# OpenMatchmaking/microservice-matchmaking

Measured on AMD Instinct MI355X. Metric: matched players/sec over 1M-player pool, higher is better.
Workload: dtype int32

## Files before the change

### microservice_matchmaking_amd/csrc/mm_engine.hip

```cpp
#include <hip/hip_runtime.h>

#include <stdint.h>
#include <stdio.h>
#include <stdlib.h>
#include <string.h>
#include <time.h>

#include <dlfcn.h>

#include <algorithm>
#include <mutex>
#include <cmath>
#include <new>
#include <vector>

#include "../../include/mm_engine.h"
#include "../../include/mm_wait.h"
#include <mm_gfx950.h>


#define MM_NO_SLOT 0xFFFFFFFFu
#define MM_ST_FREE 0
#define MM_ST_LIVE 1
#define MM_ST_CANCELLED 2
// ... 2103 lines not shown
            last_tp = tp;
            for (uint32_t g = 0; g < G; ++g) P.pyq[g] = 0;
            P.pyq[yield_g] = yield_q;
            {
                P.grp = (e->tn.pair_group_min && tiles >= e->tn.pair_group_min && tp == PK_TMAX) ? PK_GS : 0u;
                const uint32_t ngr = P.grp ? (tiles + P.grp - 1u) / P.grp : 0u;
                dim3 rgrid(tiles, G);
                P.xslots = 0;
                uint32_t tof[MM_MAX_GROUPS];
                for (uint32_t g = 0; g < G; ++g) tof[g] = P.bm[g] ? (P.bm[g] + tp - 1u) / tp : 0u;
                if (persist) {
                    const uint32_t slots = pair_xcd_map(P, tof, G, true);
                    if (slots) {
                        P.grp = 0;
                        const uint32_t K = e->tn.pair_pbatch, slice = MM_PERSIST_SLICE ? MM_PERSIST_SLICE : K + 1u;
                        for (uint32_t it = 0; it <= K; it += slice)
                            TILE_LAUNCH(kp_rounds, dim3(8u * slots), dim3(PT_THREADS), P, it, it + slice < K + 1u ? it + slice : K + 1u, K);
                        ++e->ps.pair_rounds_launches;
                        after_persist = true;
                        COMPACT_LAUNCH();
                        HIPCHK(e, hipGetLastError());
                        MMTRY(results_absorb(e, M.L));
                        MMTRY(results_send(e, sent_no, M.L, e->tn.results_early ? MM_RESULTS_MIN_PAIR : 0xFFFFFFFFu));
                        continue;
                    }
                    P.xslots = 0;
                }
                if (e->tn.pair_xcd) {
                    const uint32_t slots = pair_xcd_map(P, tof, G);
                    if (slots) rgrid = dim3(8u * slots);
                }
                uint32_t r = e->round_ctr;
                TILE_LAUNCH(kp_round, rgrid, dim3(PT_THREADS), P, r, 1u);
                ++r;
                if (P.grp) TILE_LAUNCH(kp_group, dim3(ngr, G), dim3(1024), P, r);
                for (uint32_t b = 0; b < (want_fit && e->tn.pair_batch > 12u ? 12u : e->tn.pair_batch); ++b) {
                    TILE_LAUNCH(kp_round, rgrid, dim3(PT_THREADS), P, r, 0u);
                    ++e->ps.pair_round_launches;
                    ++r;
                    if (P.grp) TILE_LAUNCH(kp_group, dim3(ngr, G), dim3(1024), P, r);
                }
                TILE_LAUNCH(kp_round_commit, dim3(tiles, G), dim3(256), P, r);
                hipLaunchKernelGGL(kp_round_stage, dim3(G), dim3(64), 0, e->stream, P, r);
                COMPACT_LAUNCH();
                e->round_ctr = r;
            }
#undef COMPACT_LAUNCH
#undef TILE_LAUNCH
            HIPCHK(e, hipGetLastError());
            MMTRY(results_absorb(e, M.L));
            MMTRY(results_send(e, sent_no, M.L, e->tn.results_early ? MM_RESULTS_MIN_PAIR : 0xFFFFFFFFu));
        }
    }
    hipLaunchKernelGGL(kp_late, dim3(G), dim3(PL_THREADS), 0, e->stream, P);
    hipLaunchKernelGGL(kp_finish, dim3(G), dim3(1024), 0, e->stream, P);
    HIPCHK(e, hipGetLastError());
    if (tail_send) {
        MMTRY(results_absorb(e, M.L));
        MMTRY(results_send(e, tail_no, M.L, e->tn.results_early ? MM_RESULTS_MIN_PAIR : 0xFFFFFFFFu));
    }
    return MM_OK;
}

static void report_team(const mm_engine* e)
{
    const uint32_t G = e->cfg.n_groups;
    for (uint32_t g = 0; g < G; ++g) {
        const TeamChain& t = e->h_tchains[g];
        const uint32_t np = t.passes + 1u;
        fprintf(stderr, "[mm-team] g%u fast %u m %u passes %u out %u left %u | cancel tick: head sat out %u, seated %u, lobby filtered %u, anchor moved %u x | "
                "kt_f, the middle chunk, cycles per pass: first loads %u, probes + lists %u, replacements %u, look-ups from scratch %u, barrier %u, step C %u; anchors at work per pass %u | "
                "F values written %u, changed after the first pass %u | kt_chase: sub-queue entries looked at by the stored lobby's fills %u, by %u look-ups %u\n",
                g, t.fast, t.m, t.passes, t.n_out, t.qlen,
                t.dbg[6] & 1u, (t.dbg[6] >> 1) & 1u, (t.dbg[6] >> 2) & 1u, t.dbg[7],
                t.tmk[0] / np, t.tmk[1] / np, t.tmk[2] / np, t.tmk[3] / np, t.tmk[4] / np, t.tmk[5] / np, t.dbg[2] / np, t.dbg[5], t.dbg[4],
                t.dbg[0], t.dbg[3], t.dbg[1]);
        if (t.lt[11])
            fprintf(stderr, "[mm-team] g%u kt_fc's chaser: %u passes, %u lobbies by F; cycles per pass: all %u, the chase loop %u, its hops by F %u, of them on kt_f's flags %u; "
                    "cycles per hop without the flags %u; %u look-ups, cycles each: starts %u, the roles' stretches %u, the members' records %u, seats + kills (the one a pass ends on) %u "
                    "(with MM_TEAM_LATE=0: kt_late keeps its own timers in the same words)\n",
                    g, t.lt[11], t.lt[12], 16u * (t.lt[9] / t.lt[11]), 16u * (t.lt[10] / t.lt[11]), 16u * (t.lt[13] / t.lt[11]), 16u * (t.lt[8] / t.lt[11]),
                    t.lt[12] ? (uint32_t)(16ull * (t.lt[13] - t.lt[8]) / t.lt[12]) : 0u,
                    t.lt[3], t.lt[3] ? 16u * (t.lt[4] / t.lt[3]) : 0u, t.lt[3] ? 16u * (t.lt[5] / t.lt[3]) : 0u, t.lt[3] ? 16u * (t.lt[6] / t.lt[3]) : 0u,
                    16u * (t.lt[7] / t.lt[11]));
    }
}

static void report_team_late(const mm_engine* e, const uint32_t* p0)
{
    const uint32_t G = e->cfg.n_groups;
    for (uint32_t g = 0; g < G; ++g) {
        const TeamChain& t = e->h_tchains[g];
        if (t.fast && t.passes != p0[g])
            fprintf(stderr, "[mm-team-late] g%u: kt_late walked passes %u..%u%s (m %u, sub-queues %u %u %u %u %u): "
                    "%u lobbies by record, %u looked up, %u left open, %u stored fills; entries scanned per role %u %u %u %u %u; "
                    "cycles/16: records %u look-ups %u fills %u ring waits %u all %u\n", g, p0[g], t.passes,
                    t.done ? "" : " and handed the chain back", t.m, t.len[0], t.len[1], t.len[2], t.len[3], t.len[4],
                    t.lt[1], t.lt[2], t.lt[3], t.lt[4], t.lt[5], t.lt[6], t.lt[7], t.lt[8], t.lt[9], t.lt[10], t.lt[11],
                    t.lt[12], t.lt[14], t.lt[13]);
    }
}

static void report_team_pass(mm_engine* e, uint32_t guard)
{
    const uint32_t G = e->cfg.n_groups;
    uint32_t gl = 0;
    for (uint32_t g = 1; g < G; ++g)
// ... 142 lines not shown
        ++e->ps.host_looks;
        {
            uint32_t fl = 0;
            for (uint32_t g = 0; g < G; ++g) if (e->h_tchains[g].fast) fl += e->h_tchains[g].flags_late;
            e->ps.team_flags_late = fl;
        }
        bool busy = false, late = late_ok;
        uint32_t most = 0;
        for (uint32_t g = 0; g < G; ++g) {
            const TeamChain& t = e->h_tchains[g];
            if (!t.fast || t.done) continue;
            busy = true;
            most = t.n_vis > most ? t.n_vis : most;
            if (t.n_vis > e->tn.team_late) late = false;
        }
        if (e->tn.debug && late_now) report_team_late(e, p0);
        if (e->tn.debug && e->tn.team_batch == 1u && !late_now) report_team_pass(e, guard);
        {
            uint32_t bf[MM_MAX_GROUPS];
            for (uint32_t g = 0; g < G; ++g) { bf[g] = e->h_tchains[g].before; team_no[g] = e->h_tchains[g].fast ? e->h_tchains[g].n_out : 0u; }
            if (!e->r_based) results_set_bases(e, bf, M.L);
            team_have = true;
        }
        if (!busy) break;
        team_order();
        if (late_now) {
            late_now = false;
            if (pass < 2u) pass = 2u;
            batch = e->tn.team_batch;
            continue;
        }
        late_now = late;
        n_emit = most / (TT_WAVES - 1u) + 1u;
        if (n_emit > e->tn.team_emit_max) n_emit = e->tn.team_emit_max;
        batch = (e->tn.team_late && most <= 3u * e->tn.team_late) ? (e->tn.team_batch < 4u ? e->tn.team_batch : 4u) : e->tn.team_batch;
    }
    if (e->ps.team_flags_late) { e->ps.team_flags_late_total += e->ps.team_flags_late; e->ps.degraded = 1; }
    hipLaunchKernelGGL(kt_fin_scatter, dim3(nch, G), dim3(TT_CH), 0, e->stream, P);
    hipLaunchKernelGGL(kt_fin_copy, dim3(nch, G), dim3(TT_CH), 0, e->stream, P);
    HIPCHK(e, hipGetLastError());
    if (e->tn.debug) report_team(e);
    return MM_OK;
}

static int report_pair(mm_engine* e)
{
    const uint32_t G = e->cfg.n_groups;
    std::vector<PairChain> hp(G);
    HIPCHK(e, hipMemcpy(hp.data(), e->d_pchains, G * sizeof(PairChain), hipMemcpyDeviceToHost));
    for (uint32_t g = 0; g < G; ++g)
        fprintf(stderr, "[mm-pair] g%u fast %u m %u qlen %u passes %u out %u rounds %u (group hops of tile 0: %u of %u entries looked at, %u not of the round) | stale %u inv %u slowsucc %u compact %u fixed(w1) %u | chase clk %u wall(100MHz) %u wrapscan clk %u\n",
                g, hp[g].fast, hp[g].m, hp[g].qlen, hp[g].passes, hp[g].n_out, hp[g].rounds, hp[g].ghops, hp[g].gtry, hp[g].gstale, hp[g].dbg[0], hp[g].dbg[1],
                hp[g].dbg[2], hp[g].dbg[3], hp[g].dbg[4], hp[g].dbg[5], hp[g].dbg[6], hp[g].dbg[7]);
    for (uint32_t g = 0; g < G; ++g)
        if (hp[g].rounds) {
            const uint32_t nr = hp[g].tm[5] ? hp[g].tm[5] : 1u;
            fprintf(stderr, "[mm-pair] g%u tile1 cycles/round over %u rounds (load %u walk+stage+sweepA %u apply %u | detect %u items %u long %u (%.1f long items) | graph %u resolve %u publish %u | cand+head %u)\n",
                    g, nr, hp[g].tm[0] / nr, hp[g].tm[6] / nr, hp[g].tm[9] / nr, hp[g].tm[1] / nr, hp[g].tm[12] / nr, hp[g].tm[2] / nr,
                    (double)hp[g].tm[11] / nr, hp[g].tm[7] / nr, hp[g].tm[8] / nr, hp[g].tm[10] / nr, hp[g].tm[4] / nr);
        }
    for (uint32_t g = 0; g < G; ++g)
        if (hp[g].ppass) {
            const uint32_t nr = hp[g].ptm[5] ? hp[g].ptm[5] : 1u;
            fprintf(stderr, "[mm-pair] g%u kp_rounds: %u passes inside persistent launches (%u launches gave up so far); tile1 cycles/pass over %u passes (barrier %u fast hops %u walk+sweepA %u apply %u | detect %u items %u long %u | graph %u resolve %u publish %u | head+arrive %u) walk loop %.0f cycles, %.1f hops\n",
                    g, hp[g].ppass, e->pair_pstops, nr, hp[g].ptm[0] / nr, hp[g].ptm[3] / nr, hp[g].ptm[6] / nr, hp[g].ptm[9] / nr, hp[g].ptm[1] / nr,
                    hp[g].ptm[12] / nr, hp[g].ptm[2] / nr, hp[g].ptm[7] / nr, hp[g].ptm[8] / nr, hp[g].ptm[10] / nr, hp[g].ptm[4] / nr,
                    16.0 * hp[g].ptm[13] / nr, (double)hp[g].ptm[15] / nr);
            fprintf(stderr, "[mm-pair] g%u kp_rounds, tile 1's walker off the fast path: %u hops whose partner had left, %.0f cycles each; %u hops without a partner inside the horizon, %.0f cycles each\n",
                    g, hp[g].pslow[0], hp[g].pslow[0] ? 16.0 * hp[g].pslow[1] / hp[g].pslow[0] : 0.0, hp[g].pslow[2],
                    hp[g].pslow[2] ? 16.0 * hp[g].pslow[3] / hp[g].pslow[2] : 0.0);
        }
    {
        fprintf(stderr, "[mm-pair] physical XCD mask of each chain's workgroups in its last kp_rounds launch:");
        for (uint32_t g = 0; g < G; ++g) fprintf(stderr, " g%u=0x%x", g, hp[g].pxm);
        fprintf(stderr, " | key %p rec %p %p bitsp %p %p pbar %p stream %p\n", (void*)e->d_pk_key[0], (void*)e->d_pk_scratch, (void*)e->d_pk_rec1,
                (void*)e->d_pk_bitsp[0], (void*)e->d_pk_bitsp[1], (void*)e->d_pk_pbar, (void*)e->stream);
    }
    if (e->tn.pair_tune & 0x10000u) {
        const uint32_t nt = 40u;
        std::vector<uint4> dg(nt);
        for (uint32_t g = 0; g < G; ++g) {
            if (!hp[g].ppass) continue;
            HIPCHK(e, hipMemcpy(dg.data(), e->d_pk_grec + (size_t)g * e->pk_gstride, nt * sizeof(uint4), hipMemcpyDeviceToHost));
            fprintf(stderr, "[mm-pair] g%u kp_rounds, cycles from barrier to arrival per tile (passes):", g);
            for (uint32_t t = 0; t < nt; ++t) if (dg[t].y && dg[t].y != 0xFFFFFFFFu) fprintf(stderr, " t%u=%u(%u)", t, dg[t].x / dg[t].y, dg[t].y);
            fprintf(stderr, "\n");
        }
    }
    if (e->tn.pair_tune & 0x2000u) {
        unsigned long long tested = 0, algo = 0;
        for (uint32_t g = 0; g < G; ++g) { tested += hp[g].tested; algo += hp[g].pairs; }
        fprintf(stderr, "[mm-pair] predicate tests the kernels physically performed (next[] build, repairs, head scans, LDS-resident walk): %llu = %.2f x the %llu pair evaluations of the reference algorithm\n",
                tested, algo ? (double)tested / (double)algo : 0.0, algo);
        std::vector<uint32_t> xc(e->pk_max_tiles);
        HIPCHK(e, hipMemcpy(xc.data(), e->d_pk_tilectl + ((size_t)TC_DISP * G + 0) * e->pk_max_tiles,
                            e->pk_max_tiles * sizeof(uint32_t), hipMemcpyDeviceToHost));
        fprintf(stderr, "[mm-pair] g0 XCD of tile 0..47's workgroup at its last round:");
        for (uint32_t t = 0; t < 48 && t < e->pk_max_tiles; ++t) fprintf(stderr, " %u", xc[t] & 0xFu);
        fprintf(stderr, "\n");
    }
    if (e->tn.pair_tune & 0x2000u)
        for (uint32_t g = 0; g < G; ++g)
            if (hp[g].rounds)
                fprintf(stderr, "[mm-pair] g%u walk loop of tile 1's workgroup: %u iterations, %.0f cycles each (%.0f cycles per timed round)\n",
                        g, hp[g].tm[15], hp[g].tm[15] ? 16.0 * hp[g].tm[13] / hp[g].tm[15] : 0.0,
                        16.0 * hp[g].tm[13] / (hp[g].tm[5] ? hp[g].tm[5] : 1u));
// ... 1078 lines not shown
```

### microservice_matchmaking_amd/csrc/mm_pair.inc

```

#define PK_NO 0xFFFFFFFFu
#define PK_ABORT 0xFFFFFFFEu

#define NX_INV 0u
#define NX_NONE 0xFFFFu
#define NX_FAR 0xFFFEu

#ifndef PK_T
#define PK_T 8192u
#endif
enum : uint32_t { PK_TMAX = PK_T };
#undef PK_T
static constexpr uint32_t PK_T = PK_TMAX;
#ifndef PK_TILES_MAX
#define PK_TILES_MAX 40u
#endif
#define PK_XSEG 4u
#ifndef PK_GS
#define PK_GS 8u
#endif
#ifndef PK_GROUP_MIN
#define PK_GROUP_MIN 64u
#endif
#ifndef PL_MAX
// ... 19 lines not shown
#define DISP_SEATED 0xFFFFFFFEu
#define REC_CLEAN 0u
#define REC_PARTNER 1u
#define REC_FAR 2u
#define REC_NONE 3u
#define EV_NONE 0u
#define EV_DONE 1u
#define EV_COMPACT 2u

struct RoundState {
    uint32_t live;
    uint32_t done;
    uint32_t want_compact, rounds;
    uint32_t qlen, passes, n_out, has_anchor;
    uint32_t a_key, a_slot, a_cons, a_team;
    int32_t  a_rating;
    uint32_t pos0;
    uint32_t changed0, extra0;
    uint32_t a_oi;
    unsigned long long pairs, scanned;
};

struct PairChain {
    uint32_t fast;
    uint32_t m;
    uint32_t qlen;
    uint32_t buf;
    int32_t  rmin;
    uint32_t has_anchor;
    uint32_t a_key, a_slot, a_cons, a_team;
    int32_t  a_rating;
    uint32_t passes, n_out, before, err;
    uint32_t pos0;
    uint32_t changed0;
    uint32_t extra0;
    unsigned long long pairs, scanned;
    unsigned long long tested;
    unsigned long long tested_nx;
    uint32_t dbg[8];
    uint32_t stage;
    uint32_t ntiles;
    uint32_t want_compact;
    uint32_t cur_pass;
    uint32_t new_m;
    uint32_t rounds;
    uint32_t ghops;
    uint32_t gtry, gstale;
    uint32_t tm[16];
    uint32_t pfail;
    uint32_t ppass;
    uint32_t pxm;
    uint32_t pslow[4];
    uint32_t ptm[16];
    RoundState rs[2];
};

struct PairParams {
    uint32_t mode, n_groups, capacity, window, eqmask;
    uint32_t out_slot_stride, out_rec_stride, bits_stride;
    uint32_t pstride;
    uint32_t tune;
    uint32_t purge;
    uint8_t* state;
    uint32_t* released;
    uint32_t* n_released;
    ChainDev* chains;
    PairChain* pchains;
    int32_t* q_rating;
    uint32_t* q_cons;
    uint32_t* q_slot;
    uint32_t* key[2];
    uint32_t* oidx[2];
    uint16_t* nx16[2];
    uint32_t* bits[2];
    uint32_t* scratch;
    uint16_t* g16;
    uint32_t* rec2[2];
    uint16_t* exa[2];
    uint32_t* bitsp[2];
    uint32_t* headp[2];
    uint4* grec;
    uint32_t grp;
    uint32_t xslots;
    uint32_t xseg[8][PK_XSEG];
    uint16_t xcnt[8][PK_XSEG];
    uint32_t gstride;
    unsigned long long* pbar;
    uint32_t* pxmask;
    uint32_t ptimeout0, ptimeout1;
    uint32_t pinject;
    uint32_t* pyield;
    uint32_t pyq[MM_MAX_GROUPS];
    uint16_t* wpre;
    uint32_t* tilectl;
    uint32_t max_tiles;
    uint32_t* out_slots;
    float* out_score;
    uint32_t* out_pass;
    uint32_t bm[MM_MAX_GROUPS];
    uint8_t bbuf[MM_MAX_GROUPS];
};

#define PK_DEAD 0x80000000u
#define PK_SPAN_BITS 19
#define PK_RMASK 0x7FFFFu
static __device__ __forceinline__ uint32_t pk_pack(int32_t r, uint32_t cons, int32_t rmin, uint32_t eqmask)
// ... 71 lines not shown
        bool fast = lb.n <= 1u && m <= max_len;
        if (m + has > 0 && ((long long)hi - (long long)lo) >= (1ll << PK_SPAN_BITS)) fast = false;
        if (m + has == 0) lo = 0;
        uint32_t pos0 = 0, changed0 = 0, extra0 = 0;
        if (fast && P.purge && has) {
            const uint32_t hs = ch->head_state;
            const uint32_t stale_slot = a_slot;
            if (hs != 0u && P.state[stale_slot] != MM_ST_LIVE) {
                if (hs == 1u) {
                    const size_t qo = (size_t)c * P.capacity;
                    const int32_t hr = qr[0];
                    const uint32_t hc = P.q_cons[qo];
                    const uint32_t d = hr >= a_rating ? (uint32_t)hr - (uint32_t)a_rating : (uint32_t)a_rating - (uint32_t)hr;
                    pos0 = 1;
                    if (d <= P.window && (((hc ^ a_cons) & P.eqmask) == 0u)) {
                        extra0 = 1; changed0 = 1;
                        a_slot = P.q_slot[qo]; a_rating = hr; a_cons = hc; team = 1u - team;
                    } else has = 0;
                } else has = 0;
                P.state[stale_slot] = MM_ST_FREE;
                P.released[atomicAdd(P.n_released, 1u)] = stale_slot;
            }
        }
        pc->fast = fast ? 1u : 0u;
        pc->m = m;
        pc->qlen = m - extra0;
        pc->pos0 = pos0;
        pc->changed0 = changed0;
        pc->extra0 = extra0;
        pc->buf = 0;
        pc->rmin = lo;
        pc->has_anchor = has;
        pc->a_key = has ? pk_pack(a_rating, a_cons, lo, P.eqmask) : 0u;
        pc->a_slot = a_slot;
        pc->a_cons = a_cons;
        pc->a_team = team;
        pc->a_rating = a_rating;
        pc->passes = 0;
        pc->n_out = 0;
        pc->before = m + lb.n + (P.purge ? ch->purged : 0u);
        pc->err = 0;
        pc->pairs = 0;
        pc->scanned = 0;
        pc->tested = 0;
        pc->tested_nx = 0;
        for (int k = 0; k < 8; ++k) pc->dbg[k] = 0;
        pc->stage = m < PL_MAX ? PS_LATE : PS_TILED;
        pc->ntiles = (m + PK_T - 1u) / PK_T;
        pc->want_compact = 0;
        pc->cur_pass = 0;
        pc->new_m = m;
        pc->rounds = 0;
        pc->ghops = 0; pc->gtry = 0; pc->gstale = 0;
        for (int k = 0; k < 16; ++k) { pc->tm[k] = 0; pc->ptm[k] = 0; }
        pc->pfail = 0; pc->ppass = 0;
        for (int k = 0; k < 4; ++k) pc->pslow[k] = 0;
        pc->pxm = 0;
        P.pbar[g] = 0ull; P.pxmask[g] = 0u;
        if (g == 0u) *P.pyield = 0u;
    }
    if (m <= max_len) {
        const uint32_t nt = (m + PK_T - 1u) / PK_T;
        for (uint32_t t = tid; t < P.max_tiles; t += 1024) {
            P.tilectl[((size_t)TC_ENT * P.n_groups + g) * P.max_tiles + t] = PK_NO;
            P.tilectl[((size_t)TC_ALIVE * P.n_groups + g) * P.max_tiles + t] =
                t < nt ? dev_min_u32(PK_T, m - t * PK_T) : 0u;
        }
    }
}

__global__ __launch_bounds__(1024) void kp_pack(PairParams P)
{
    const uint32_t g = blockIdx.y;
    const PairChain* const pc = P.pchains + g;
    if (!pc->fast) return;
    const uint32_t m = pc->m;
    const uint32_t i = blockIdx.x * 1024u + threadIdx.x;
    const uint32_t c = P.mode * P.n_groups + g;
    const size_t qo = (size_t)c * P.capacity, po = (size_t)g * P.pstride;
    if (i < m) {
        P.key[0][po + i] = pk_pack(P.q_rating[qo + i], P.q_cons[qo + i], pc->rmin, P.eqmask);
        P.oidx[0][po + i] = i;
        P.nx16[0][po + i] = (uint16_t)NX_INV;
    }
    if ((i & 31u) == 0u && i < m + 32u) {
        const uint32_t left = i < m ? m - i : 0u;
        uint32_t wbits = left >= 32u ? 0xFFFFFFFFu : ((1u << left) - 1u);
        if (i == 0u && pc->extra0) wbits &= ~1u;
        P.bits[0][(size_t)g * P.bits_stride + (i >> 5)] = wbits;
    }
}

#define NXI_THREADS 512
#define NXI_SEG 2048u
#define NXI_STAGE 8192u
__global__ __launch_bounds__(NXI_THREADS) void kp_nx_init(PairParams P, uint32_t seg, uint32_t stage)
{
    __shared__ uint32_t s_k[NXI_STAGE];
    const uint32_t g = blockIdx.y;
    const PairChain* const pc = P.pchains + g;
    if (!pc->fast) return;
    const uint32_t m = pc->m;
    const uint32_t s0 = blockIdx.x * seg;
    if (s0 >= m) return;
    const int tid = threadIdx.x, lane = tid & 63, wave = tid >> 6;
    const size_t po = (size_t)g * P.pstride;
    const uint32_t* const key = P.key[0] + po;
// ... 90 lines not shown
        for (; p + 256u <= end; p += 256u) {
            uint32_t kv[4];
#pragma unroll
            for (uint32_t u = 0; u < 4u; ++u) kv[u] = lds_ld(key + p + 64u * u + (uint32_t)lane);
#pragma unroll
            for (uint32_t u = 0; u < 4u; ++u) {
                const unsigned long long b = __ballot(pk_in(kv[u], klo, krng));
                if (b) return p + 64u * u + (uint32_t)__ffsll(b) - 1u;
            }
        }
    }
    if (ev) {
        for (; p + 256u <= end; p += 256u) {
            uint32_t kv[4];
#pragma unroll
            for (uint32_t u = 0; u < 4u; ++u) kv[u] = lds_ld(key + p + 64u * u + (uint32_t)lane);
            const uint32_t e = lds_ld(ev);
#pragma unroll
            for (uint32_t u = 0; u < 4u; ++u) {
                const unsigned long long b = __ballot(pk_in(kv[u], klo, krng));
                if (b) return p + 64u * u + (uint32_t)__ffsll(b) - 1u;
            }
            if (uni(e) != EV_NONE) return PK_ABORT;
        }
    }
    for (; p < end; p += 64u) {
        const uint32_t c = p + (uint32_t)lane;
        const bool ok = c < end && pk_in(lds_ld(key + c), klo, krng);
        const unsigned long long b = __ballot(ok);
        if (b) return p + (uint32_t)__ffsll(b) - 1u;
        if (ev && lds_ld(ev) != EV_NONE) return PK_ABORT;
    }
    return PK_NO;
}

static __device__ __forceinline__ uint32_t l_succ(const uint32_t* bits, uint32_t pos, uint32_t m, int lane)
{
    if (pos >= m) return PK_NO;
    const uint32_t nwords = (m + 31u) >> 5, w0 = pos >> 5;
    for (uint32_t wb = w0; wb < nwords; wb += 64u) {
        const uint32_t wi = wb + (uint32_t)lane;
        uint32_t v = wi < nwords ? lds_ld(bits + wi) : 0u;
        if (wi == w0) v &= 0xFFFFFFFFu << (pos & 31u);
        const unsigned long long b = __ballot(v != 0u);
        if (b) {
            const int l = __ffsll(b) - 1;
            const uint32_t vv = lane_get(v, l);
            return ((wb + (uint32_t)l) << 5) + (uint32_t)__ffs((int)vv) - 1u;
        }
    }
    return PK_NO;
}

#define PL_RING 512u
#define PL_EXT 0xFFFEu
#define PL_NOPART 0xFFFFu
#define PL_S (PL_MAX - 1u)
#define PL_SPEC 64u

static __device__ __forceinline__ uint32_t nxg_make(uint32_t t, uint32_t gi) { return t | ((gi << 2) << 16); }

static __device__ __forceinline__ uint32_t lane_succ(const uint32_t* bits, uint32_t from, uint32_t nwords)
{
    uint32_t wi = from >> 5;
    if (wi >= nwords) return PL_S;
    uint32_t v = lds_ld(bits + wi) & (0xFFFFFFFFu << (from & 31u));
    while (v == 0u) {
        if (++wi >= nwords) return PL_S;
        v = lds_ld(bits + wi);
    }
    return (wi << 5) + (uint32_t)__ffs((int)v) - 1u;
}

__global__ __launch_bounds__(PL_THREADS) void kp_late(PairParams P)
{
    __shared__ uint32_t s_path[PL_SPEC];
    __shared__ uint32_t s_nxg[PL_MAX];
    __shared__ uint32_t s_key[PL_MAX];
    __shared__ uint32_t s_bits[PL_WORDS + 64];
    __shared__ uint16_t s_wpre[PL_WORDS];
    __shared__ uint32_t s_ring[PL_RING];
    __shared__ uint16_t s_ringp[PL_RING];
    __shared__ uint32_t s_wtot[16];
    __shared__ uint32_t s_event, s_m, s_head, s_tail, s_killed, s_aidx, s_buf, s_nout;
    __shared__ uint32_t s_ext[5];

    const int tid = threadIdx.x, lane = tid & 63, wave = tid >> 6;
    const uint32_t g = blockIdx.x;
    PairChain* const pc = P.pchains + g;
    if (!pc->fast || pc->stage != PS_LATE) return;
    const uint32_t c = P.mode * P.n_groups + g;
    const size_t qo = (size_t)c * P.capacity, po = (size_t)g * P.pstride;
    const uint32_t w = P.window;
    uint32_t* const os = P.out_slots + (size_t)g * P.out_slot_stride;
    float* const osc = P.out_score + (size_t)g * P.out_rec_stride;
    uint32_t* const opass = P.out_pass + (size_t)g * P.out_rec_stride;
    uint32_t* const vbits = s_bits;
    uint32_t* const vev = &s_event;

    uint32_t m = pc->m;
    const uint32_t pass0 = pc->passes;
    {
        const uint32_t nwords = (m + 31u) >> 5;
        for (uint32_t i = tid; i < PL_WORDS + 64u; i += PL_THREADS)
            s_bits[i] = i < nwords ? P.bits[pc->buf][(size_t)g * P.bits_stride + i] : 0u;
        const uint32_t* const key = P.key[pc->buf] + po;
        __syncthreads();
        for (uint32_t i = tid; i < m; i += PL_THREADS) s_key[i] = key[i] | (l_alive(s_bits, i) ? 0u : PK_DEAD);
        if (tid == 0) {
            s_event = EV_NONE; s_m = m; s_head = 0; s_tail = 0; s_killed = 0; s_aidx = PK_NO; s_buf = pc->buf;
            s_ext[0] = pc->a_slot; s_ext[1] = (uint32_t)pc->a_rating; s_ext[2] = pc->a_cons;
            s_ext[3] = pc->a_key; s_ext[4] = pc->a_team;
        }
        __syncthreads();
        for (uint32_t i = tid; i < PL_MAX; i += PL_THREADS) {
            uint32_t t = LNX_NONE, gi = PL_S;
            if (i < m) {
                const uint32_t o = P.nx16[pc->buf][po + i];
                t = o == NX_NONE ? LNX_NONE : (o == NX_INV || o == NX_FAR) ? LNX_INV : i + o;
                if (t < LNX_INV) gi = lane_succ(s_bits, t + 1u, nwords);
            }
            s_nxg[i] = nxg_make(t, gi);
        }
    }
    __syncthreads();

    uint32_t has_anchor = pc->has_anchor, a_idx = PL_EXT, a_pushed = 1;
    uint32_t qlen = pc->qlen, pos = pc->pos0, passes = pc->passes, in_pass = pc->pos0 ? 1u : 0u, changed = pc->changed0;
    uint32_t n_out = pc->n_out;
    unsigned long long pairs = pc->pairs, scanned = pc->scanned;
    if (pc->pos0) { scanned += qlen + pc->extra0; pairs += qlen + pc->extra0; }
    uint32_t rk = 0, rtail = 0;
    uint32_t emit_idx = pc->n_out;
    uint32_t d_stale = 0, d_inv = 0, d_slowsucc = 0, d_compact = 0, d_fixed = 0, d_clk = 0, d_wall = 0, d_wrapc = 0;
    unsigned long long d_tst = 0;
    const uint32_t fix_waves = 13u - dev_min_u32(P.tune & 15u, 13u);
    const uint32_t fix_sleep = (P.tune >> 4) & 0xFFu;

#define RING_ROOM(N)                                                                        \
    do {                                                                                    \
        if (rk - rtail + (N) > PL_RING) {                                                   \
            rtail = uni(lds_ld(&s_tail));                                                   \
            while (rk - rtail + (N) > PL_RING) { __builtin_amdgcn_s_sleep(2); rtail = uni(lds_ld(&s_tail)); } \
        }                                                                                   \
    } while (0)
#define RING_PUSH(A, T)                                                                     \
    do {                                                                                    \
        RING_ROOM(1u);                                                                      \
        if (lane == 0) {                                                                    \
            s_ring[rk % PL_RING] = (A) | ((T) << 16);                                       \
            s_ringp[rk % PL_RING] = (uint16_t)(passes - pass0);                             \
        }                                                                                   \
        ++rk;                                                                               \
        if (lane == 0) lds_st(&s_head, rk);                                                 \
    } while (0)
#define RING_DRAIN()    \
    do {                                                                                    \
        uint32_t kd = uni(lds_ld(&s_killed));                                               \
        while (kd != rk) { __builtin_amdgcn_s_sleep(1); kd = uni(lds_ld(&s_killed)); }      \
    } while (0)

    for (;;) {
        if (wave == 0) {
            __builtin_amdgcn_s_setprio(3);
            uint32_t ev = EV_NONE;
            const long long tc0 = clock64(), tw0 = wall_clock64();
            for (;;) {
                if (!in_pass) {
                    RING_DRAIN();
                    if (qlen == 0u) { ev = EV_DONE; break; }
                    if (m > PL_COMPACT_MIN && qlen * 2u < m) { ev = EV_COMPACT; break; }
                    in_pass = 1; pos = 0; changed = 0;
                    scanned += qlen;
                    pairs += qlen;
                }
                uint32_t t = PK_NO;
                if (!has_anchor) {
                    const uint32_t a = uni(l_succ(vbits, pos, m, lane));
                    if (a == PK_NO) {
                        ++passes; in_pass = 0;
                        if (!changed) { ev = EV_DONE; break; }
                        continue;
                    }
                    --qlen; --pairs; changed = 1; has_anchor = 1; a_idx = a; a_pushed = 0;
                    pos = a + 1u;
                } else {
                    const long long ts = clock64();
                    const uint32_t a_key = a_idx == PL_EXT ? s_ext[3] : (s_key[a_idx] & ~PK_DEAD);
                    t = uni(l_scan_fit(s_key, a_key, pos, m, w, lane, nullptr));
                    d_tst += (t == PK_NO ? m : t) - pos;
                    d_wrapc += (uint32_t)(clock64() - ts);
                    if (t == PK_NO) {
                        ++passes; in_pass = 0;
                        if (!changed) { ev = EV_DONE; break; }
                        continue;
                    }
                }
                for (;;) {
                    bool blind = t == PK_NO && a_idx != PL_EXT;
                    if (blind) {
                        const uint32_t r0 = uni(lds_ld(s_nxg + a_idx));
                        blind = (r0 & 0xFFFFu) < LNX_INV && (r0 >> 18) != PL_S;
                    }
                    if (blind) {
                        uint32_t x4 = a_idx << 2;
                        for (uint32_t k0 = 0; k0 < PL_SPEC; k0 += 8u) {
#pragma unroll
                            for (uint32_t k = 0; k < 8u; ++k) {
                                const uint32_t r = lds_ld((const uint32_t*)((const char*)s_nxg + x4));
                                s_path[k0 + k] = r;
                                x4 = r >> 16;
                            }
                            if (uni(x4) == (PL_S << 2)) {
                                for (uint32_t k = k0 + 8u + (uint32_t)lane; k < PL_SPEC; k += 64u) s_path[k] = nxg_make(LNX_NONE, PL_S);
                                break;
                            }
                        }
                        const uint32_t r = s_path[lane];
                        const uint32_t rp = lane ? s_path[lane - 1] : 0u;
                        const uint32_t ia = lane ? (rp >> 18) : a_idx;
                        const uint32_t it = r & 0xFFFFu, ig = r >> 18;
                        bool ok = ia != PL_S && it < LNX_INV && ig != PL_S;
                        if (ok) ok = l_alive(vbits, it) && l_alive(vbits, ig);
                        const unsigned long long good = __ballot(ok);
                        const uint32_t ns = good == ~0ull ? 64u : (uint32_t)__ffsll(~good) - 1u;
                        if (ns) {
                            RING_ROOM(ns);
                            if ((uint32_t)lane < ns) {
                                s_ring[(rk + (uint32_t)lane) % PL_RING] = ia | (it << 16);
                                s_ringp[(rk + (uint32_t)lane) % PL_RING] = (uint16_t)(passes - pass0);
                            }
                            rk += ns;
                            if (lane == 0) lds_st(&s_head, rk);
                            qlen -= 2u * ns; pairs -= ns; n_out += ns; changed = 1;
                            a_idx = lane_get(ig, (int)ns - 1);
                            a_pushed = 0;
                        }
                        if (ns == PL_SPEC) continue;
                    }
                    const uint32_t a_key = a_idx == PL_EXT ? s_ext[3] : (s_key[a_idx] & ~PK_DEAD);
                    if (t == PK_NO) {
                        const uint32_t cnx = uni(lds_ld(s_nxg + a_idx)) & 0xFFFFu;
                        if (cnx == LNX_NONE) break;
                        if (cnx < LNX_INV && l_alive(vbits, cnx)) t = cnx;
                        else {
                            if (cnx == LNX_INV) ++d_inv; else ++d_stale;
                            t = uni(l_scan_fit(s_key, a_key, cnx == LNX_INV ? a_idx + 1u : cnx + 1u, m, w, lane, nullptr));
                            d_tst += (t == PK_NO ? m : t) - (cnx == LNX_INV ? a_idx + 1u : cnx + 1u);
                            if (t == PK_NO) break;
                        }
                    }
                    RING_PUSH(a_idx, t);
                    --qlen; changed = 1; has_anchor = 0; pos = t + 1u; ++n_out;
                    ++d_slowsucc;
                    const uint32_t a2 = uni(l_succ(vbits, t + 1u, m, lane));
                    if (a2 == PK_NO) break;
                    --qlen; --pairs; has_anchor = 1; a_idx = a2; a_pushed = 0;
                    pos = a2 + 1u;
                    t = PK_NO;
                }
                if (has_anchor && !a_pushed) { RING_PUSH(a_idx, PL_NOPART); a_pushed = 1; }
                ++passes; in_pass = 0;
                if (!changed) { ev = EV_DONE; break; }
            }
            d_clk += (uint32_t)(clock64() - tc0);
            d_wall += (uint32_t)(wall_clock64() - tw0);
            if (lane == 0) { s_aidx = has_anchor ? a_idx : PK_NO; s_nout = n_out; lds_st(vev, ev); }
            __builtin_amdgcn_s_setprio(0);
        } else if (wave == 1) {
            uint32_t ktail = uni(lds_ld(&s_killed));
            for (;;) {
                uint32_t head = uni(lds_ld(&s_head));
                if (head == ktail) {
                    if (lds_ld(vev) != EV_NONE) {
                        head = uni(lds_ld(&s_head));
                        if (head == ktail) break;
                    } else { __builtin_amdgcn_s_sleep(1); continue; }
                }
                const uint32_t nb = dev_min_u32(64u, head - ktail);
                if ((uint32_t)lane < nb) {
                    const uint32_t e = s_ring[(ktail + (uint32_t)lane) % PL_RING];
                    const uint32_t a = e & 0xFFFFu, t = e >> 16;
                    if (a != PL_EXT) { atomicAnd(&s_bits[a >> 5], ~(1u << (a & 31u))); atomicOr(&s_key[a], PK_DEAD); }
                    if (t != PL_NOPART) { atomicAnd(&s_bits[t >> 5], ~(1u << (t & 31u))); atomicOr(&s_key[t], PK_DEAD); }
                }
                wave_lockstep();
                ktail += nb;
                if (lane == 0) lds_st(&s_killed, ktail);
            }
        } else if (wave == 2) {
            uint32_t tail = uni(lds_ld(&s_tail));
            const uint32_t* const oidx = P.oidx[uni(lds_ld(&s_buf))] + po;
            for (;;) {
                const uint32_t killed = uni(lds_ld(&s_killed));
                if (killed == tail) {
                    if (lds_ld(vev) != EV_NONE && uni(lds_ld(&s_head)) == tail && uni(lds_ld(&s_killed)) == tail) break;
                    __builtin_amdgcn_s_sleep(2);
                    continue;
                }
                const uint32_t nb = dev_min_u32(64u, killed - tail);
                const bool mine = (uint32_t)lane < nb;
                const uint32_t slotr = (tail + (uint32_t)lane) % PL_RING;
                const uint32_t e = mine ? s_ring[slotr] : 0xFFFFFFFFu;
                const uint32_t a = e & 0xFFFFu, t = e >> 16;
                const bool is_match = mine && t != PL_NOPART;
                const unsigned long long mm = __ballot(is_match);
                if (is_match) {
                    const uint32_t k = emit_idx + (uint32_t)__popcll(mm & ((1ull << lane) - 1ull));
                    const uint32_t ka = a == PL_EXT ? s_ext[3] : s_key[a];
                    const uint32_t kt = s_key[t];
                    const uint32_t ra = pk_rating(ka), rt = pk_rating(kt);
                    const uint32_t team = a == PL_EXT ? s_ext[4] : 0u;
                    os[2u * k + team] = a == PL_EXT ? s_ext[0] : P.q_slot[qo + oidx[a]];
                    os[2u * k + (1u - team)] = P.q_slot[qo + oidx[t]];
                    osc[k] = (float)(int32_t)(ra > rt ? ra - rt : rt - ra);
// ... 75 lines not shown
        {
            const uint32_t nwords = (m + 31u) >> 5;
            const uint32_t pcw = (uint32_t)tid < nwords ? (uint32_t)__popc(s_bits[tid]) : 0u;
            const uint32_t incl = wave_incl_scan(pcw, lane);
            if (lane == 63) s_wtot[wave] = incl;
            __syncthreads();
            if ((uint32_t)tid < PL_WORDS) {
                uint32_t off = 0;
                for (int x = 0; x < wave; ++x) off += s_wtot[x];
                s_wpre[tid] = (uint16_t)(off + incl - pcw);
            }
            __syncthreads();
            uint32_t* const oidx_new = P.oidx[cur ^ 1u] + po;
            for (uint32_t base = 0; base < m; base += PL_THREADS) {
                const uint32_t i = base + (uint32_t)tid;
                uint32_t r = PK_NO, nk = 0, nv = 0, no = 0;
                if (i < m && l_alive(s_bits, i)) {
                    const uint32_t bw = s_bits[i >> 5];
                    r = s_wpre[i >> 5] + (uint32_t)__popc(bw & ((1u << (i & 31u)) - 1u));
                    nk = s_key[i];
                    const uint32_t v = s_nxg[i];
                    uint32_t t = v & 0xFFFFu, gi = v >> 18;
                    if (t < LNX_INV) {
                        if (l_alive(s_bits, t)) {
                            t = s_wpre[t >> 5] + (uint32_t)__popc(s_bits[t >> 5] & ((1u << (t & 31u)) - 1u));
                            if (gi != PL_S && l_alive(s_bits, gi))
                                gi = s_wpre[gi >> 5] + (uint32_t)__popc(s_bits[gi >> 5] & ((1u << (gi & 31u)) - 1u));
                            else gi = PL_S;
                        } else { t = LNX_INV; gi = PL_S; }
                    } else gi = PL_S;
                    nv = nxg_make(t, gi);
                    no = oidx[i];
                }
                __syncthreads();
                if (r != PK_NO) { s_key[r] = nk; s_nxg[r] = nv; oidx_new[r] = no; }
                __syncthreads();
            }
            const uint32_t nm = (uint32_t)s_wpre[nwords - 1u] + (uint32_t)__popc(s_bits[nwords - 1u]);
            __syncthreads();
            for (uint32_t i = tid; i < PL_WORDS; i += PL_THREADS) {
                const uint32_t lo = i << 5;
                s_bits[i] = lo + 32u <= nm ? 0xFFFFFFFFu : (lo < nm ? (1u << (nm - lo)) - 1u : 0u);
            }
            for (uint32_t i = nm + (uint32_t)tid; i < m; i += PL_THREADS) s_nxg[i] = nxg_make(LNX_NONE, PL_S);
            if (tid == 0) { s_m = nm; s_buf = cur ^ 1u; s_event = EV_NONE; s_aidx = PK_NO; }
            __syncthreads();
            m = s_m;
            ++d_compact;
        }
    }
#undef RING_ROOM
#undef RING_PUSH
#undef RING_DRAIN

    {
        const uint32_t nwords = (m + 31u) >> 5;
        for (uint32_t i = tid; i < nwords; i += PL_THREADS) P.bits[s_buf][(size_t)g * P.bits_stride + i] = s_bits[i];
        if (tid == 0) {
            pc->stage = PS_DONE;
            pc->pos0 = 0; pc->changed0 = 0; pc->extra0 = 0;
            pc->m = m;
            pc->qlen = qlen;
            pc->buf = s_buf;
            pc->has_anchor = has_anchor;
            if (has_anchor) {
                pc->a_key = s_ext[3];
                pc->a_slot = s_ext[0];
                pc->a_cons = s_ext[2];
                pc->a_team = s_ext[4];
                pc->a_rating = (int32_t)s_ext[1];
            }
            pc->passes = passes;
            pc->n_out = n_out;
            pc->pairs = pairs;
            pc->scanned = scanned;
            pc->dbg[0] = d_stale;
            pc->dbg[1] = d_inv;
            pc->dbg[2] = d_slowsucc;
            pc->dbg[3] = d_compact;
            pc->dbg[5] = d_clk;
            pc->dbg[6] = d_wall;
            pc->dbg[7] = d_wrapc;
        }
        if (tid == 128 && emit_idx != s_nout) atomicOr(&pc->err, MM_ERRF_SEAT_INVARIANT);
        if (tid == 192) pc->dbg[4] = d_fixed;
        if ((P.tune & 0x2000u) && lane == 0 && d_tst) atomicAdd(&pc->tested, d_tst);
    }
}

#define PT_THREADS 1024
#define PW_WAVES 0
#define PF_N 6u

static __device__ __forceinline__ uint32_t* tc_row(const PairParams& P, uint32_t row, uint32_t g)
{
    return P.tilectl + ((size_t)row * P.n_groups + g) * P.max_tiles;
}

static __device__ __forceinline__ uint32_t rec_make(uint32_t kind, uint32_t cnt, uint32_t land)
{
    return (kind << 30) | (cnt << 17) | land;
}

static __device__ __forceinline__ void copy_words_x4(uint32_t* dst, const uint32_t* src, uint32_t n, int tid, int nthreads)
{
    const uint4* const s4 = (const uint4*)src;
    uint4* const d4 = (uint4*)dst;
    for (uint32_t i = tid; i < (n + 3u) >> 2; i += nthreads) d4[i] = s4[i];
}


template <uint32_t TP>
static __device__ __forceinline__ void prep_stage_keys(uint32_t* s_key, const uint32_t* s_bits, const uint32_t* gkey,
                                                       uint32_t hl, int tid, int nthreads = PT_THREADS)
{
    constexpr uint32_t PK_T = TP;
    (void)PK_T;
    constexpr uint32_t STG_T = PT_THREADS - 64u * (1u + PW_WAVES);
    constexpr uint32_t STG = ((2u * PK_T + 64u) / 4u + STG_T - 1u) / STG_T;
    const uint32_t ngroups = (hl + 64u + 3u) >> 2;
    uint4 k[STG];
#pragma unroll
    for (uint32_t j = 0; j < STG; ++j) {
        const uint32_t i4 = (uint32_t)tid + j * (uint32_t)nthreads;
        if (i4 < ngroups && (i4 << 2) < hl) k[j] = ((const uint4*)gkey)[i4];
        else k[j] = uint4{0xFFFFFFFFu, 0xFFFFFFFFu, 0xFFFFFFFFu, 0xFFFFFFFFu};
    }
#pragma unroll
    for (uint32_t j = 0; j < STG; ++j) {
        const uint32_t i4 = (uint32_t)tid + j * (uint32_t)nthreads;
        if (i4 >= ngroups) continue;
        const uint32_t i = i4 << 2;
        const uint32_t nib = (s_bits[i >> 5] >> (i & 31u)) & 0xFu;
        uint4 q = k[j];
        q.x = i + 0u < hl ? (q.x | ((nib & 1u) ? 0u : PK_DEAD)) : 0xFFFFFFFFu;
        q.y = i + 1u < hl ? (q.y | ((nib & 2u) ? 0u : PK_DEAD)) : 0xFFFFFFFFu;
        q.z = i + 2u < hl ? (q.z | ((nib & 4u) ? 0u : PK_DEAD)) : 0xFFFFFFFFu;
        q.w = i + 3u < hl ? (q.w | ((nib & 8u) ? 0u : PK_DEAD)) : 0xFFFFFFFFu;
        ((uint4*)s_key)[i4] = q;
    }
}
// ... 1713 lines not shown
```

Measured before the change: 107.1 million.

## Restructure kp_late chaser walk with cached anchor keys and batched liveness checks

Rewrites the late-stage pair chaser loop. It caches the anchor key across steps and reuses the cut-point's next/liveness word instead of re-reading it. It unrolls the first eight speculative path hops and then walks in PL_BLOCK chunks, checks liveness with branch-free loads, and prefetches the successor bit words before the ring push. It also adds a templated timed variant with per-phase cycle counters, selected by a tune bit. The intent is to cut LDS round-trips and serial dependency latency in the single-wave chaser, at the cost of more complex state that could go stale.

```diff
diff --git a/microservice_matchmaking_amd/csrc/mm_engine.hip b/microservice_matchmaking_amd/csrc/mm_engine.hip
--- a/microservice_matchmaking_amd/csrc/mm_engine.hip
+++ b/microservice_matchmaking_amd/csrc/mm_engine.hip
@@ -2179,7 +2179,8 @@
             MMTRY(results_send(e, sent_no, M.L, e->tn.results_early ? MM_RESULTS_MIN_PAIR : 0xFFFFFFFFu));
         }
     }
-    hipLaunchKernelGGL(kp_late, dim3(G), dim3(PL_THREADS), 0, e->stream, P);
+    if (e->tn.pair_tune & 0x20000u) hipLaunchKernelGGL(kp_late_timed, dim3(G), dim3(PL_THREADS), 0, e->stream, P);
+    else hipLaunchKernelGGL(kp_late, dim3(G), dim3(PL_THREADS), 0, e->stream, P);
     hipLaunchKernelGGL(kp_finish, dim3(G), dim3(1024), 0, e->stream, P);
     HIPCHK(e, hipGetLastError());
     if (tail_send) {
@@ -2428,6 +2429,23 @@
         fprintf(stderr, "[mm-pair] g%u fast %u m %u qlen %u passes %u out %u rounds %u (group hops of tile 0: %u of %u entries looked at, %u not of the round) | stale %u inv %u slowsucc %u compact %u fixed(w1) %u | chase clk %u wall(100MHz) %u wrapscan clk %u\n",
                 g, hp[g].fast, hp[g].m, hp[g].qlen, hp[g].passes, hp[g].n_out, hp[g].rounds, hp[g].ghops, hp[g].gtry, hp[g].gstale, hp[g].dbg[0], hp[g].dbg[1],
                 hp[g].dbg[2], hp[g].dbg[3], hp[g].dbg[4], hp[g].dbg[5], hp[g].dbg[6], hp[g].dbg[7]);
+    if (e->tn.pair_tune & 0x20000u) {
+        uint32_t gl = 0;
+        for (uint32_t g = 1; g < G; ++g) if (hp[g].ltm[13] > hp[gl].ltm[13]) gl = g;
+        const uint32_t* const L = hp[gl].ltm;
+        if (hp[gl].fast && L[13]) {
+            const double np = L[13], nl = L[14] ? L[14] : 1u;
+            const uint32_t total = hp[gl].dbg[5], scan = hp[gl].dbg[7];
+            const uint32_t sum = L[0] + scan + L[3] + L[6] + L[9] + L[10] + L[11];
+            const uint32_t part[8] = {L[0], scan, L[3], L[6], L[9], L[10], L[11], total >= sum ? total - sum : 0u};
+            static const char* const name[8] = {"drain", "headscan", "blind", "check+handover", "careful word/key", "careful rescan", "careful succ+push", "bookkeeping"};
+            fprintf(stderr, "[mm-pair] g%u kp_late chaser: %u passes %u lobbies, %u cycles = %.0f a pass, %.0f a lobby; cycles total / a pass / a lobby / share:", gl, L[13], L[14], total, total / np, total / nl);
+            for (int k = 0; k < 8; ++k)
+                fprintf(stderr, " %s %u / %.0f / %.1f / %.1f%%%s", name[k], part[k], part[k] / np, part[k] / nl, total ? 100.0 * part[k] / total : 0.0, k < 7 ? " |" : "");
+            fprintf(stderr, " || counts: passes begun %u, head scans %u, blind reads %u (%u on the sentinel, %.0f cycles a read), checks %u, waits for ring room %u, careful steps %u (stale %u inv %u), seated-anchor pushes %u\n",
+                    L[1], L[2], L[4], L[5], L[4] ? (double)L[3] / L[4] : 0.0, L[7], L[8], L[12], hp[gl].dbg[0], hp[gl].dbg[1], L[15]);
+        }
+    }
     for (uint32_t g = 0; g < G; ++g)
         if (hp[g].rounds) {
             const uint32_t nr = hp[g].tm[5] ? hp[g].tm[5] : 1u;
diff --git a/microservice_matchmaking_amd/csrc/mm_pair.inc b/microservice_matchmaking_amd/csrc/mm_pair.inc
--- a/microservice_matchmaking_amd/csrc/mm_pair.inc
+++ b/microservice_matchmaking_amd/csrc/mm_pair.inc
@@ -95,6 +95,7 @@
     uint32_t pxm;
     uint32_t pslow[4];
     uint32_t ptm[16];
+    uint32_t ltm[16];
     RoundState rs[2];
 };
 
@@ -272,7 +273,7 @@
         pc->new_m = m;
         pc->rounds = 0;
         pc->ghops = 0; pc->gtry = 0; pc->gstale = 0;
-        for (int k = 0; k < 16; ++k) { pc->tm[k] = 0; pc->ptm[k] = 0; }
+        for (int k = 0; k < 16; ++k) { pc->tm[k] = 0; pc->ptm[k] = 0; pc->ltm[k] = 0; }
         pc->pfail = 0; pc->ppass = 0;
         for (int k = 0; k < 4; ++k) pc->pslow[k] = 0;
         pc->pxm = 0;
@@ -469,11 +470,35 @@
     return PK_NO;
 }
 
+static __device__ __forceinline__ uint32_t l_succ_ld(const uint32_t* bits, uint32_t pos, uint32_t m, int lane)
+{
+    const uint32_t nwords = (m + 31u) >> 5, wi = (pos >> 5) + (uint32_t)lane;
+    return pos < m && wi < nwords ? lds_ld(bits + wi) : 0u;
+}
+static __device__ __forceinline__ uint32_t l_succ_from(const uint32_t* bits, uint32_t pos, uint32_t m, int lane, uint32_t v)
+{
+    if (pos >= m) return PK_NO;
+    const uint32_t w0 = pos >> 5;
+    if (lane == 0) v &= 0xFFFFFFFFu << (pos & 31u);
+    const unsigned long long b = __ballot(v != 0u);
+    if (b) {
+        const int l = __ffsll(b) - 1;
+        const uint32_t vv = lane_get(v, l);
+        return ((w0 + (uint32_t)l) << 5) + (uint32_t)__ffs((int)vv) - 1u;
+    }
+    return l_succ(bits, (w0 + 64u) << 5, m, lane);
+}
+
 #define PL_RING 512u
 #define PL_EXT 0xFFFEu
 #define PL_NOPART 0xFFFFu
 #define PL_S (PL_MAX - 1u)
 #define PL_SPEC 64u
+#ifndef PL_BLOCK
+#define PL_BLOCK 8u
+#endif
+#define CW_NONE 0xFFFFFFFFu
+#define CW_ASK 2u
 
 static __device__ __forceinline__ uint32_t nxg_make(uint32_t t, uint32_t gi) { return t | ((gi << 2) << 16); }
 
@@ -489,7 +514,8 @@
     return (wi << 5) + (uint32_t)__ffs((int)v) - 1u;
 }
 
-__global__ __launch_bounds__(PL_THREADS) void kp_late(PairParams P)
+template <bool LTM>
+static __device__ __forceinline__ void late_walk(const PairParams& P)
 {
     __shared__ uint32_t s_path[PL_SPEC];
     __shared__ uint32_t s_nxg[PL_MAX];
@@ -501,6 +527,7 @@
     __shared__ uint32_t s_wtot[16];
     __shared__ uint32_t s_event, s_m, s_head, s_tail, s_killed, s_aidx, s_buf, s_nout;
     __shared__ uint32_t s_ext[5];
+    __shared__ uint32_t s_lt[16];
 
     const int tid = threadIdx.x, lane = tid & 63, wave = tid >> 6;
     const uint32_t g = blockIdx.x;
@@ -525,6 +552,7 @@
         __syncthreads();
         for (uint32_t i = tid; i < m; i += PL_THREADS) s_key[i] = key[i] | (l_alive(s_bits, i) ? 0u : PK_DEAD);
         if (tid == 0) {
+            for (int k = 0; k < 16; ++k) s_lt[k] = 0u;
             s_event = EV_NONE; s_m = m; s_head = 0; s_tail = 0; s_killed = 0; s_aidx = PK_NO; s_buf = pc->buf;
             s_ext[0] = pc->a_slot; s_ext[1] = (uint32_t)pc->a_rating; s_ext[2] = pc->a_cons;
             s_ext[3] = pc->a_key; s_ext[4] = pc->a_team;
@@ -543,6 +571,7 @@
     __syncthreads();
 
     uint32_t has_anchor = pc->has_anchor, a_idx = PL_EXT, a_pushed = 1;
+    uint32_t a_kv = 0, a_kok = 0;
     uint32_t qlen = pc->qlen, pos = pc->pos0, passes = pc->passes, in_pass = pc->pos0 ? 1u : 0u, changed = pc->changed0;
     uint32_t n_out = pc->n_out;
     unsigned long long pairs = pc->pairs, scanned = pc->scanned;
@@ -553,11 +582,18 @@
     unsigned long long d_tst = 0;
     const uint32_t fix_waves = 13u - dev_min_u32(P.tune & 15u, 13u);
     const uint32_t fix_sleep = (P.tune >> 4) & 0xFFu;
+    constexpr bool ltmr = LTM;
+    const uint32_t n_out0 = pc->n_out;
+    uint32_t lt0 = 0;
+#define LT_ON() do { if (ltmr) lt0 = (uint32_t)clock64(); } while (0)
+#define LT_OFF(K) do { if (ltmr) { const uint32_t lt1 = (uint32_t)clock64(); if (lane == 0) atomicAdd(&s_lt[K], lt1 - lt0); } } while (0)
+#define LT_CNT(K, N) do { if (ltmr && lane == 0) atomicAdd(&s_lt[K], (uint32_t)(N)); } while (0)
 
 #define RING_ROOM(N)                                                                        \
     do {                                                                                    \
         if (rk - rtail + (N) > PL_RING) {                                                   \
             rtail = uni(lds_ld(&s_tail));                                                   \
+            if (rk - rtail + (N) > PL_RING) LT_CNT(8, 1u);                                  \
             while (rk - rtail + (N) > PL_RING) { __builtin_amdgcn_s_sleep(2); rtail = uni(lds_ld(&s_tail)); } \
         }                                                                                   \
     } while (0)
@@ -584,7 +620,10 @@
             const long long tc0 = clock64(), tw0 = wall_clock64();
             for (;;) {
                 if (!in_pass) {
+                    LT_ON();
                     RING_DRAIN();
+                    LT_OFF(0);
+                    LT_CNT(1, 1u);
                     if (qlen == 0u) { ev = EV_DONE; break; }
                     if (m > PL_COMPACT_MIN && qlen * 2u < m) { ev = EV_COMPACT; break; }
                     in_pass = 1; pos = 0; changed = 0;
@@ -599,85 +638,130 @@
                         if (!changed) { ev = EV_DONE; break; }
                         continue;
                     }
-                    --qlen; --pairs; changed = 1; has_anchor = 1; a_idx = a; a_pushed = 0;
+                    --qlen; --pairs; changed = 1; has_anchor = 1; a_idx = a; a_pushed = 0; a_kok = 0;
                     pos = a + 1u;
                 } else {
                     const long long ts = clock64();
-                    const uint32_t a_key = a_idx == PL_EXT ? s_ext[3] : (s_key[a_idx] & ~PK_DEAD);
-                    t = uni(l_scan_fit(s_key, a_key, pos, m, w, lane, nullptr));
+                    if (!a_kok) { a_kv = a_idx == PL_EXT ? s_ext[3] : s_key[a_idx]; a_kok = 1; }
+                    t = uni(l_scan_fit(s_key, uni(a_kv) & ~PK_DEAD, pos, m, w, lane, nullptr));
                     d_tst += (t == PK_NO ? m : t) - pos;
                     d_wrapc += (uint32_t)(clock64() - ts);
+                    LT_CNT(2, 1u);
                     if (t == PK_NO) {
                         ++passes; in_pass = 0;
                         if (!changed) { ev = EV_DONE; break; }
                         continue;
                     }
                 }
+                uint32_t cw = CW_NONE, cw_live = CW_ASK, cw_fresh = 0;
                 for (;;) {
-                    bool blind = t == PK_NO && a_idx != PL_EXT;
-                    if (blind) {
-                        const uint32_t r0 = uni(lds_ld(s_nxg + a_idx));
-                        blind = (r0 & 0xFFFFu) < LNX_INV && (r0 >> 18) != PL_S;
-                    }
-                    if (blind) {
-                        uint32_t x4 = a_idx << 2;
-                        for (uint32_t k0 = 0; k0 < PL_SPEC; k0 += 8u) {
-#pragma unroll
-                            for (uint32_t k = 0; k < 8u; ++k) {
-                                const uint32_t r = lds_ld((const uint32_t*)((const char*)s_nxg + x4));
-                                s_path[k0 + k] = r;
+                    if (t == PK_NO && a_idx != PL_EXT && cw == CW_NONE) {
+                        LT_ON();
+                        uint32_t r = lds_ld(s_nxg + a_idx);
+                        cw = uni(r); cw_live = CW_ASK; cw_fresh = 1;
+                        if ((cw & 0xFFFFu) < LNX_INV && (cw >> 18) != PL_S) {
+                            uint32_t x4 = r >> 16, kn = 8u;
+                            s_path[0] = r;
+#pragma unroll
+                            for (uint32_t k = 1u; k < 8u; ++k) {
+                                r = lds_ld((const uint32_t*)((const char*)s_nxg + x4));
+                                s_path[k] = r;
                                 x4 = r >> 16;
                             }
-                            if (uni(x4) == (PL_S << 2)) {
-                                for (uint32_t k = k0 + 8u + (uint32_t)lane; k < PL_SPEC; k += 64u) s_path[k] = nxg_make(LNX_NONE, PL_S);
-                                break;
+                            if (uni(x4) != (PL_S << 2)) {
+                                for (; kn < PL_SPEC; ) {
+#pragma unroll
+                                    for (uint32_t k = 0; k < PL_BLOCK; ++k) {
+                                        r = lds_ld((const uint32_t*)((const char*)s_nxg + x4));
+                                        s_path[kn + k] = r;
+                                        x4 = r >> 16;
+                                    }
+                                    kn += PL_BLOCK;
+                                    if (uni(x4) == (PL_S << 2)) break;
+                                }
+                            }
+                            for (uint32_t k = kn + (uint32_t)lane; k < PL_SPEC; k += 64u) s_path[k] = nxg_make(LNX_NONE, PL_S);
+                            LT_OFF(3);
+                            LT_CNT(4, kn);
+                            LT_ON();
+                            const uint32_t rl = s_path[lane];
+                            const uint32_t rp = lane ? s_path[lane - 1] : 0u;
+                            const uint32_t ia = lane ? (rp >> 18) : a_idx;
+                            const uint32_t it = rl & 0xFFFFu, ig = rl >> 18;
+                            if (ltmr) { const uint32_t nsent = (uint32_t)__popcll(__ballot(ia == PL_S && (uint32_t)lane < kn)); LT_CNT(5, nsent); }
+                            const bool pt = ia != PL_S && it < LNX_INV, pg = pt && ig != PL_S;
+                            const uint32_t jt = pt ? it : 0u, jg = pg ? ig : 0u;
+                            const uint32_t wt = lds_ld(vbits + (jt >> 5)), wg = lds_ld(vbits + (jg >> 5));
+                            const uint32_t live_t = pt ? (wt >> (jt & 31u)) & 1u : 0u;
+                            const bool ok = pg && live_t && ((wg >> (jg & 31u)) & 1u);
+                            const unsigned long long good = __ballot(ok);
+                            const uint32_t ns = good == ~0ull ? 64u : (uint32_t)__ffsll(~good) - 1u;
+                            if (ns) {
+                                RING_ROOM(ns);
+                                if ((uint32_t)lane < ns) {
+                                    s_ring[(rk + (uint32_t)lane) % PL_RING] = ia | (it << 16);
+                                    s_ringp[(rk + (uint32_t)lane) % PL_RING] = (uint16_t)(passes - pass0);
+                                }
+                                rk += ns;
+                                if (lane == 0) lds_st(&s_head, rk);
+                                qlen -= 2u * ns; pairs -= ns; n_out += ns; changed = 1;
+                                a_idx = lane_get(ig, (int)ns - 1);
+                                a_pushed = 0; a_kok = 0;
+                            }
+                            if (ns == PL_SPEC) { cw = CW_NONE; LT_OFF(6); LT_CNT(7, 1u); continue; }
+                            cw = lane_get(rl, (int)ns); cw_live = lane_get(live_t, (int)ns); cw_fresh = 0;
+                            LT_OFF(6);
+                            LT_CNT(7, 1u);
+                        } else LT_OFF(9);
+                    }
+                    LT_ON();
+                    LT_CNT(12, 1u);
+                    if (t == PK_NO) {
+                        uint32_t cnx = cw & 0xFFFFu;
+                        if (cnx == LNX_NONE) { LT_OFF(9); break; }
+                        if (cnx < LNX_INV && cw_live == CW_ASK) cw_live = uni(l_alive(vbits, cnx));
+                        if (cnx < LNX_INV && cw_live) { t = cnx; LT_OFF(9); }
+                        else {
+                            if (!cw_fresh) {
+                                cnx = uni(lds_ld(s_nxg + a_idx)) & 0xFFFFu;
+                                if (cnx == LNX_NONE) { LT_OFF(9); break; }
+                                if (cnx < LNX_INV && uni(l_alive(vbits, cnx))) t = cnx;
+                            }
+                            if (!a_kok) { a_kv = a_idx == PL_EXT ? s_ext[3] : s_key[a_idx]; a_kok = 1; }
+                            LT_OFF(9);
+                            if (t == PK_NO) {
+                                LT_ON();
+                                if (cnx == LNX_INV) ++d_inv; else ++d_stale;
+                                t = uni(l_scan_fit(s_key, uni(a_kv) & ~PK_DEAD, cnx == LNX_INV ? a_idx + 1u : cnx + 1u, m, w, lane, nullptr));
+                                d_tst += (t == PK_NO ? m : t) - (cnx == LNX_INV ? a_idx + 1u : cnx + 1u);
+                                LT_OFF(10);
+                                if (t == PK_NO) break;
                             }
                         }
-                        const uint32_t r = s_path[lane];
-                        const uint32_t rp = lane ? s_path[lane - 1] : 0u;
-                        const uint32_t ia = lane ? (rp >> 18) : a_idx;
-                        const uint32_t it = r & 0xFFFFu, ig = r >> 18;
-                        bool ok = ia != PL_S && it < LNX_INV && ig != PL_S;
-                        if (ok) ok = l_alive(vbits, it) && l_alive(vbits, ig);
-                        const unsigned long long good = __ballot(ok);
-                        const uint32_t ns = good == ~0ull ? 64u : (uint32_t)__ffsll(~good) - 1u;
-                        if (ns) {
-                            RING_ROOM(ns);
-                            if ((uint32_t)lane < ns) {
-                                s_ring[(rk + (uint32_t)lane) % PL_RING] = ia | (it << 16);
-                                s_ringp[(rk + (uint32_t)lane) % PL_RING] = (uint16_t)(passes - pass0);
-                            }
-                            rk += ns;
-                            if (lane == 0) lds_st(&s_head, rk);
-                            qlen -= 2u * ns; pairs -= ns; n_out += ns; changed = 1;
-                            a_idx = lane_get(ig, (int)ns - 1);
-                            a_pushed = 0;
-                        }
-                        if (ns == PL_SPEC) continue;
-                    }
-                    const uint32_t a_key = a_idx == PL_EXT ? s_ext[3] : (s_key[a_idx] & ~PK_DEAD);
-                    if (t == PK_NO) {
-                        const uint32_t cnx = uni(lds_ld(s_nxg + a_idx)) & 0xFFFFu;
-                        if (cnx == LNX_NONE) break;
-                        if (cnx < LNX_INV && l_alive(vbits, cnx)) t = cnx;
-                        else {
-                            if (cnx == LNX_INV) ++d_inv; else ++d_stale;
-                            t = uni(l_scan_fit(s_key, a_key, cnx == LNX_INV ? a_idx + 1u : cnx + 1u, m, w, lane, nullptr));
-                            d_tst += (t == PK_NO ? m : t) - (cnx == LNX_INV ? a_idx + 1u : cnx + 1u);
-                            if (t == PK_NO) break;
-                        }
-                    }
+                    } else LT_OFF(9);
+                    LT_ON();
+                    RING_ROOM(1u);
+                    const uint32_t sv = l_succ_ld(vbits, t + 1u, m, lane);
                     RING_PUSH(a_idx, t);
                     --qlen; changed = 1; has_anchor = 0; pos = t + 1u; ++n_out;
                     ++d_slowsucc;
-                    const uint32_t a2 = uni(l_succ(vbits, t + 1u, m, lane));
+                    const uint32_t a2 = uni(l_succ_from(vbits, t + 1u, m, lane, sv));
+                    LT_OFF(11);
                     if (a2 == PK_NO) break;
-                    --qlen; --pairs; has_anchor = 1; a_idx = a2; a_pushed = 0;
+                    --qlen; --pairs; has_anchor = 1; a_idx = a2; a_pushed = 0; a_kok = 0;
                     pos = a2 + 1u;
-                    t = PK_NO;
-                }
-                if (has_anchor && !a_pushed) { RING_PUSH(a_idx, PL_NOPART); a_pushed = 1; }
+                    t = PK_NO; cw = CW_NONE;
+                }
+                if (has_anchor && !a_pushed) {
+                    LT_ON();
+                    if (!a_kok && a_idx != PL_EXT) { a_kv = s_key[a_idx]; a_kok = 1; }
+                    RING_PUSH(a_idx, PL_NOPART);
+                    a_pushed = 1;
+                    LT_OFF(11);
+                    LT_CNT(15, 1u);
+                }
                 ++passes; in_pass = 0;
+                LT_CNT(13, 1u);
                 if (!changed) { ev = EV_DONE; break; }
             }
             d_clk += (uint32_t)(clock64() - tc0);
@@ -859,6 +943,9 @@
 #undef RING_ROOM
 #undef RING_PUSH
 #undef RING_DRAIN
+#undef LT_ON
+#undef LT_OFF
+#undef LT_CNT
 
     {
         const uint32_t nwords = (m + 31u) >> 5;
@@ -888,12 +975,19 @@
             pc->dbg[5] = d_clk;
             pc->dbg[6] = d_wall;
             pc->dbg[7] = d_wrapc;
+            if (ltmr) {
+                s_lt[14] = n_out - n_out0;
+                for (int k = 0; k < 16; ++k) pc->ltm[k] = s_lt[k];
+            }
         }
         if (tid == 128 && emit_idx != s_nout) atomicOr(&pc->err, MM_ERRF_SEAT_INVARIANT);
         if (tid == 192) pc->dbg[4] = d_fixed;
         if ((P.tune & 0x2000u) && lane == 0 && d_tst) atomicAdd(&pc->tested, d_tst);
     }
 }
+
+__global__ __launch_bounds__(PL_THREADS) void kp_late(PairParams P) { late_walk<false>(P); }
+__global__ __launch_bounds__(PL_THREADS) void kp_late_timed(PairParams P) { late_walk<true>(P); }
 
 #define PT_THREADS 1024
 #define PW_WAVES 0
```

Measured after the change: 106.3 million. Within noise of the previous version (-0.8%).
